# lucasnewman/f5-tts-mlx

Hardware: AMD Instinct MI355X
Metric: mel_frames_per_sec (higher is better)
Workload: dtype f16 (IEEE-half MFMA operands, fp32 accumulate / residual stream / LayerNorm / softmax state; meets the 1e-3 gate); 1 GPU; BASELINE configs[1]: F5-TTS 335M, 32-point euler (=62 DiT forwards, CFG), batch 1/GPU x 10 s (N=937) utterances, hipGraph=True; f16 (IEEE half) MFMA operands IN PLACE OF BASELINE's bf16 -- same width and MFMA rate, three more significand bits; plain bf16 fails the 1e-3 parity gate, see sub.b1_bf16; global_batch=1, seq_len=937, parallelism=dp1 (utterance sharding)

## Files before the change

f5_tts_mlx_amd/csrc/attention.hip:

```cpp
#include "attention.hpp"

namespace F5_NS {

__device__ __forceinline__ bool attn_block_map(const F5AttnArgs& p, int qrows, int& bh, int& qblk) {
    if (gridDim.y != 1) {
        bh = blockIdx.y;
        qblk = blockIdx.x;
        return true;
    }
    const int nqb = (p.seq_len + qrows - 1) / qrows;
    const int s = blockIdx.x >> 3;
    qblk = s % nqb;
    bh = (s / nqb) * 8 + (blockIdx.x & 7);
    return bh < p.B * p.H;
}

template <bool SCALE>
__device__ __forceinline__ void attn_pin_args(const F5AttnArgs& p) {
    if (SCALE)
        asm volatile("" ::"s"(p.qk[0]), "s"(p.vt[0]), "s"(p.out[0]), "s"(p.kv_len), "s"(p.B), "s"(p.H), "s"(p.seq_len), "s"(p.npad), "s"(p.ldqk),
                     "s"(p.ldo), "s"(p.dmodel), "s"(p.scale), "s"(p.out8));
    else
        asm volatile("" ::"s"(p.qk[0]), "s"(p.vt[0]), "s"(p.out[0]), "s"(p.kv_len), "s"(p.B), "s"(p.H), "s"(p.seq_len), "s"(p.npad), "s"(p.ldqk),
                     "s"(p.ldo), "s"(p.dmodel), "s"(p.out8));
// ... 775 lines not shown
    }

#define A2P_STEP(PH)                                                                                                    \
    if (j < T) {                                                                                                        \
        A2P_WAIT_TOP(j)                                                                                                 \
        attn_barrier();                                                                                                 \
        A2P_ISSUE_GROUP(j)                                                                                              \
        const int nv_ = kvlen - j * 64;                                                                                 \
         \
        attn2p_half<((PH) + 1) & 3, 0, (PH), 0>(ak, av, qf, fr_a, fr_b, s_a, s_b, o, mneg, p_b, p_a, l_run, hi, nv_);       \
        attn2p_half<((PH) + 1) & 3, 1, (PH), 1>(ak, av, qf, fr_b, fr_a, s_b, s_a, o, mneg, p_a, p_b, l_run, hi, nv_ - 32);  \
        ++j;                                                                                                            \
    }
    {
        int j = 0;
        for (int g = (T + 3) >> 2; g > 0; --g) {
            A2P_STEP(0)
            A2P_STEP(1)
            A2P_STEP(2)
            A2P_STEP(3)
        }
    }
#undef A2P_STEP
    {
        const uint32_t stv = (uint32_t)((T - 1) & 3) * (ATTN2P_TILE * 2);
        uint32_t avf[4];
#pragma unroll
        for (int i = 0; i < 4; ++i) avf[i] = av[i] + stv;
        a2p_load_frag<4, 0, 0, 0, 1>(fr_a[0], ak, avf);
        a2p_load_frag<5, 0, 0, 0, 1>(fr_a[1], ak, avf);
        a2p_load_frag<6, 0, 0, 0, 1>(fr_a[2], ak, avf);
        a2p_load_frag<7, 0, 0, 0, 1>(fr_a[3], ak, avf);
        asm volatile("s_waitcnt lgkmcnt(0)" : "+a"(fr_a[0]), "+a"(fr_a[1]), "+a"(fr_a[2]), "+a"(fr_a[3]));
#pragma unroll
        for (int g = 0; g < 4; ++g) {
            const int sp = g >> 1, db = g & 1;
#pragma unroll
            for (int qb = 0; qb < 2; ++qb) {
                const op16x8 pb = __builtin_bit_cast(op16x8, u32x4{p_b[qb][4 * sp], p_b[qb][4 * sp + 1], p_b[qb][4 * sp + 2], p_b[qb][4 * sp + 3]});
                a2p_mfma_o(o[qb][db], fr_a[g], pb);
            }
        }
    }
#undef A2P_WAIT_TOP
#undef A2P_ISSUE_GROUP
#undef A2P_ISSUE_V
#undef A2P_ISSUE_K
    asm volatile(A2P_PAD : "+a"(o[0][0]), "+a"(o[0][1]), "+a"(o[1][0]), "+a"(o[1][1]));

#pragma unroll
    for (int qb = 0; qb < 2; ++qb) attn_store_block<false>(p, o[qb], l_run[qb], rowbase, q0 + qb * 32 + lq, h, hi);
}

template <bool HP, int KS, int NST, bool FAST = false>
__global__ __launch_bounds__(256 * KS, 1) void f5_attn2s_kernel(F5AttnArgs p) {
    constexpr int NP = HP ? 2 : 1;
    constexpr int TILE = 64 * 64;
    constexpr int RING = NST * NP * 2 * TILE;
    static_assert(KS * RING * 2 <= 160 * 1024, "LDS budget");
    static_assert((KS - 1) * 4 * 34 * 64 * 4 <= KS * RING * 2, "merge area must fit in the rings");
    __shared__ __attribute__((aligned(16))) op16_t smem_all[KS * RING];

    attn_pin_args<true>(p);
    const int tid = threadIdx.x, lane = tid & 63;
    const int wave_all = __builtin_amdgcn_readfirstlane(tid >> 6);
    const int grp = wave_all >> 2, wave = wave_all & 3;
    const int tg = tid & 255;
    op16_t* smem = smem_all + grp * RING;
    const int hi = lane >> 5, lq = lane & 31;
    int bh, qblk;
    if (!attn_block_map(p, 128, bh, qblk)) return;
    const int b = bh / p.H, h = bh - b * p.H;
    const int q0 = qblk * 128 + wave * 32;
    const int kvlen = p.kv_len ? p.kv_len[b] : p.seq_len;
    const int ntile = (kvlen + 63) >> 6;
    const int nit = (ntile + KS - 1) / KS;
    const int ntg = ntile > grp ? (ntile - grp + KS - 1) / KS : 0;
    const size_t rowbase = (size_t)b * p.seq_len;

    op16x8 qf[NP][4];
    {
        int qr = q0 + lq;
        if (qr > p.seq_len - 1) qr = p.seq_len - 1;
#pragma unroll
        for (int pp = 0; pp < NP; ++pp)
#pragma unroll
            for (int ks = 0; ks < 4; ++ks)
                qf[pp][ks] = *reinterpret_cast<const op16x8*>(p.qk[pp] + (rowbase + qr) * p.ldqk + h * 64 + ks * 16 + hi * 8);
    }

    const op16_t* kptr[NP][2];
    const op16_t* vptr[NP][2];
    int krow[2], kcol[2], ldsoff[2];
#pragma unroll
    for (int i = 0; i < 2; ++i) {
        const int q_ = i * 256 + tg;
        const int srow = q_ >> 3;
        const int schunk = (q_ & 7) ^ ((srow >> 1) & 7);
        krow[i] = attn_kperm(srow);
        kcol[i] = p.dmodel + h * 64 + schunk * 8;
        ldsoff[i] = (i * 256 + wave * 64) * 8;
#pragma unroll
        for (int pp = 0; pp < NP; ++pp) {
            kptr[pp][i] = p.qk[pp] + (rowbase + grp * 64 + krow[i]) * p.ldqk + kcol[i];
            vptr[pp][i] = p.vt[pp] + ((size_t)bh * 64 + srow) * p.npad + grp * 64 + schunk * 8;
        }
    }
    const size_t kstep = (size_t)64 * KS * p.ldqk;
#define A2S_ISSUE(jj_)                                                                                       \
    {                                                                                                        \
        op16_t* st_ = smem + ((jj_) % NST) * (NP * 2 * TILE);                                                \
        const int gt_ = (jj_) * KS + grp;                                                                    \
        const bool tail_ = (gt_ * 64 + 63) > p.seq_len - 1;                                                  \
        _Pragma("unroll") for (int i = 0; i < 2; ++i) {                                                      \
            _Pragma("unroll") for (int pp = 0; pp < NP; ++pp) {                                              \
                const op16_t* ks_ = kptr[pp][i];                                                             \
                if (tail_) {                                                                                 \
                    int key_ = gt_ * 64 + krow[i];                                                           \
                    if (key_ > p.seq_len - 1) key_ = p.seq_len - 1;                                          \
                    ks_ = p.qk[pp] + (rowbase + key_) * p.ldqk + kcol[i];                                    \
                }                                                                                            \
                attn_glds16(ks_, st_ + (pp * 2) * TILE + ldsoff[i]);                                         \
                attn_glds16(vptr[pp][i], st_ + (pp * 2 + 1) * TILE + ldsoff[i]);                             \
                kptr[pp][i] += kstep;                                                                        \
                vptr[pp][i] += 64 * KS;                                                                      \
            }                                                                                                \
        }                                                                                                    \
    }

    f32x16 o[2];
#pragma unroll
    for (int e = 0; e < 16; ++e) {
        o[0][e] = 0.0f;
        o[1][e] = 0.0f;
    }
    float m_run = -INFINITY, l_run = 0.0f;
    const float c2 = p.q_prescaled ? 1.0f : p.scale * 1.4426950408889634f;

    if (ntg > 0) A2S_ISSUE(0);
    if (NST == 3 && ntg > 1) A2S_ISSUE(1);
    ATTN_PIN_Q(qf, NP, 4);

    for (int jj = 0; jj < nit; ++jj) {
        attn_wait_barrier(NST == 3 && jj + 1 < ntg);
        if (jj + NST - 1 < ntg) A2S_ISSUE(jj + NST - 1);
        if (jj >= ntg) continue;

        const op16_t* st = smem + (jj % NST) * (NP * 2 * TILE);
        const op16_t* sK = st;
        const op16_t* sV = st + TILE;
        const op16_t* sKl = st + (NP - 1) * 2 * TILE;
        const op16_t* sVl = st + (NP - 1) * 2 * TILE + TILE;

        f32x16 s[2];
        const int key0 = (jj * KS + grp) * 64;
#define A2S_QK()                                                                                             \
        {                                                                                                    \
            __builtin_amdgcn_s_setprio(1);                                                                   \
            _Pragma("unroll") for (int kb = 0; kb < 2; ++kb) {                                               \
                _Pragma("unroll") for (int e = 0; e < 16; ++e) s[kb][e] = 0.0f;                              \
                _Pragma("unroll") for (int ks = 0; ks < 4; ++ks) {                                           \
                    const int off = attn_swz(kb * 32 + lq, ks * 2 + hi);                                     \
                    const op16x8 a = *reinterpret_cast<const op16x8*>(&sK[off]);                             \
                    s[kb] = F5_MFMA32(a, qf[0][ks], s[kb], 0, 0, 0);                                         \
                    if (HP) {                                                                                \
                        const op16x8 al = *reinterpret_cast<const op16x8*>(&sKl[off]);                       \
                        s[kb] = F5_MFMA32(al, qf[0][ks], s[kb], 0, 0, 0);                                    \
                        s[kb] = F5_MFMA32(a, qf[NP - 1][ks], s[kb], 0, 0, 0);                                \
                    }                                                                                        \
                }                                                                                            \
            }                                                                                                \
            __builtin_amdgcn_s_setprio(0);                                                                   \
            if (key0 + 64 > kvlen) {                                                                         \
                _Pragma("unroll") for (int kb = 0; kb < 2; ++kb)                                             \
                    _Pragma("unroll") for (int r = 0; r < 16; ++r) {                                         \
                        const int key = key0 + kb * 32 + 16 * hi + r;                                        \
                        if (key >= kvlen) s[kb][r] = -INFINITY;                                              \
                    }                                                                                        \
            }                                                                                                \
        }
        A2S_QK();
        float psum = 0.0f;
        bool slow = !FAST || HP || jj == 0;
        if (!slow) {
            const float mc = m_run * c2;
            attn_f32x2 ps2 = {0.0f, 0.0f};
            ps2 = attn_exp_block(s[0], c2, mc, ps2);
            ps2 = attn_exp_block(s[1], c2, mc, ps2);
            psum = ps2[0] + ps2[1];
            slow = __any(!(psum <= ATTN_SUM_LIMIT));
            if (slow) A2S_QK();
        }
        if (slow) {
            float tmax = -INFINITY;
#pragma unroll
            for (int kb = 0; kb < 2; ++kb)
#pragma unroll
                for (int r = 0; r < 16; ++r) tmax = fmaxf(tmax, s[kb][r]);
            tmax = fmaxf(tmax, __shfl_xor(tmax, 32, 64));
            if (__any(tmax > m_run)) {
                const float m_new = fmaxf(m_run, tmax);
                const float alpha = __builtin_amdgcn_exp2f((m_run - m_new) * c2);
                m_run = m_new;
                l_run *= alpha;
#pragma unroll
                for (int e = 0; e < 16; ++e) {
                    o[0][e] *= alpha;
                    o[1][e] *= alpha;
                }
            }
            const float mc = m_run * c2;
            attn_f32x2 ps2 = {0.0f, 0.0f};
            ps2 = attn_exp_block(s[0], c2, mc, ps2);
            ps2 = attn_exp_block(s[1], c2, mc, ps2);
            psum = ps2[0] + ps2[1];
        }
        l_run += psum;
#undef A2S_QK

#pragma unroll
        for (int ks4 = 0; ks4 < 4; ++ks4) {
            const int kb = ks4 >> 1, sp = ks4 & 1;
            uint32_t pw[4], pwl[4];
#pragma unroll
            for (int e = 0; e < 4; ++e) {
                const float p0 = s[kb][8 * sp + 2 * e], p1 = s[kb][8 * sp + 2 * e + 1];
                pw[e] = f5_pack2_bounded(p0, p1);
                if (HP) pwl[e] = f5_pack2_lo(p0, p1);
            }
            const op16x8 pb = __builtin_bit_cast(op16x8, u32x4{pw[0], pw[1], pw[2], pw[3]});
            op16x8 pbl = pb;
            if (HP) pbl = __builtin_bit_cast(op16x8, u32x4{pwl[0], pwl[1], pwl[2], pwl[3]});
            __builtin_amdgcn_s_setprio(1);
#pragma unroll
            for (int db = 0; db < 2; ++db) {
                const int voff = attn_swz(db * 32 + lq, 4 * kb + 2 * hi + sp);
                const op16x8 a = *reinterpret_cast<const op16x8*>(&sV[voff]);
                o[db] = F5_MFMA32(a, pb, o[db], 0, 0, 0);
                if (HP) {
                    const op16x8 al = *reinterpret_cast<const op16x8*>(&sVl[voff]);
                    o[db] = F5_MFMA32(al, pb, o[db], 0, 0, 0);
                    o[db] = F5_MFMA32(a, pbl, o[db], 0, 0, 0);
                }
            }
            __builtin_amdgcn_s_setprio(0);
        }
    }
#undef A2S_ISSUE

    __syncthreads();
    float* mrg = reinterpret_cast<float*>(smem_all);
    if (HP || !p.out8) {
        constexpr int Q = 32 / KS, NPK = 2 + 32 - Q;
        constexpr int SLD = 64 + 8;
        static_assert(KS * 4 * NPK * 64 * 4 + (HP ? 0 : 128 * SLD * 2) <= KS * RING * 2, "merge area + output staging fit in the rings");
        float* mine = mrg + (size_t)((grp * 4 + wave) * NPK) * 64 + lane;
        mine[0] = m_run;
        mine[64] = l_run;
#pragma unroll
        for (int g = 0; g < KS; ++g)
            if (grp == g) {
#pragma unroll
                for (int i = 0; i < 32; ++i)
                    if (i / Q != g) mine[(2 + (i < g * Q ? i : i - Q)) * 64] = o[i >> 4][i & 15];
            }
        __syncthreads();
        const float* src[KS];
        float mg[KS];
#pragma unroll
        for (int g = 0; g < KS; ++g) {
            src[g] = mrg + (size_t)((g * 4 + wave) * NPK) * 64 + lane;
            mg[g] = src[g][0];
        }
        float m_all = mg[0];
#pragma unroll
        for (int g = 1; g < KS; ++g) m_all = fmaxf(m_all, mg[g]);
        float ag[KS];
#pragma unroll
        for (int g = 0; g < KS; ++g) ag[g] = __builtin_amdgcn_exp2f((mg[g] - m_all) * c2);
        float l_all = __builtin_fmaf(src[0][64], ag[0], src[1][64] * ag[1]);
#pragma unroll
        for (int g = 2; g < KS; ++g) l_all = __builtin_fmaf(src[g][64], ag[g], l_all);
        float own[Q];
#pragma unroll
        for (int g = 0; g < KS; ++g)
            if (grp == g) {
#pragma unroll
                for (int j = 0; j < Q; ++j) {
                    const int i = g * Q + j;
                    float w[KS];
#pragma unroll
                    for (int k = 0; k < KS; ++k) {
                        w[k] = ag[k];
                        asm volatile("" : "+v"(w[k]));
                    }
                    float x[KS];
#pragma unroll
                    for (int k = 0; k < KS; ++k) x[k] = k == g ? o[i >> 4][i & 15] : src[k][(2 + (i < k * Q ? i : i - Q)) * 64];
                    float acc;
                    if (KS == 2) {
// ... 44 lines not shown
#pragma unroll
        for (int db = 0; db < 2; ++db)
#pragma unroll
            for (int e = 0; e < 16; ++e) dst[(2 + db * 16 + e) * 64] = o[db][e];
    }
    __syncthreads();
    if (grp > 0) return;
    float m_all = m_run;
#pragma unroll
    for (int g = 1; g < KS; ++g) m_all = fmaxf(m_all, mrg[(size_t)((g - 1) * 4 + wave) * 34 * 64 + lane]);
    {
        const float a0 = __builtin_amdgcn_exp2f((m_run - m_all) * c2);
        l_run *= a0;
#pragma unroll
        for (int e = 0; e < 16; ++e) {
            o[0][e] *= a0;
            o[1][e] *= a0;
        }
    }
#pragma unroll
    for (int g = 1; g < KS; ++g) {
        const float* src = mrg + (size_t)((g - 1) * 4 + wave) * 34 * 64 + lane;
        const float ag = __builtin_amdgcn_exp2f((src[0] - m_all) * c2);
        l_run += src[64] * ag;
#pragma unroll
        for (int db = 0; db < 2; ++db)
#pragma unroll
            for (int e = 0; e < 16; ++e) o[db][e] += src[(2 + db * 16 + e) * 64] * ag;
    }

    const float l_tot = l_run + __shfl_xor(l_run, 32, 64);
    const float inv = 1.0f / l_tot;
    const int qr = q0 + lq;
    if (!HP && p.out8) {
        if (qr < p.seq_len) attn_store_f8(p, o, inv, rowbase + qr, h, hi);
    } else if (qr < p.seq_len) {
#pragma unroll
        for (int db = 0; db < 2; ++db)
#pragma unroll
            for (int rg = 0; rg < 4; ++rg) {
                const int d = db * 32 + 8 * rg + 4 * hi;
                const float v0 = o[db][rg * 4 + 0] * inv, v1 = o[db][rg * 4 + 1] * inv;
                const float v2 = o[db][rg * 4 + 2] * inv, v3 = o[db][rg * 4 + 3] * inv;
                const size_t off = (rowbase + qr) * p.ldo + h * 64 + d;
                *reinterpret_cast<u32x2*>(p.out[0] + off) = u32x2{f5_pack2_bounded(v0, v1), f5_pack2_bounded(v2, v3)};
                if (HP && p.out[1])
                    *reinterpret_cast<u32x2*>(p.out[1] + off) = u32x2{f5_pack2_lo(v0, v1), f5_pack2_lo(v2, v3)};
            }
    }
}

int f5_attn_wide = -1;
int f5_attn_kvsplit = -1;
int f5_attn_pipe = 0;

static dim3 attn_grid(const F5AttnArgs& a, int qrows) {
    const int nqb = f5_cdiv(a.seq_len, qrows);
    return dim3(nqb * 8 * f5_cdiv(a.B * a.H, 8), 1);
}

static F5AttnKernel attn_route(const F5AttnArgs& a) {
    int ks = f5_attn_kvsplit;
    if (ks < 0) {
        const long wgs = (long)f5_cdiv(a.seq_len, 128) * a.B * a.H;
        const int ntile = f5_cdiv(a.seq_len, 64);
        ks = (wgs <= 160 && ntile >= 8) ? 4 : ((wgs <= 320 && ntile >= 4) ? 2 : 1);
    }
    if (!a.hp && ks <= 1 &&
        (f5_attn_wide >= 1 || (f5_attn_wide < 0 && (long)f5_cdiv(a.seq_len, 256) * a.B * a.H >= 512))) {
        const bool pipe = (a.pipe < 0 ? f5_attn_pipe : a.pipe) && a.q_prescaled;
        return pipe ? F5A_V2P : (a.q_prescaled ? F5A_V2F_PRE : F5A_V2F);
    }
    if (ks > 1) return a.hp ? F5A_V2S_HP : (ks >= 4 ? F5A_V2S_KS4 : F5A_V2S_KS2);
    return a.hp ? F5A_V2_HP : F5A_V2;
}

static int attn_launch(const F5AttnArgs& a, hipStream_t stream, int& reached) {
    F5_REQUIRE(a.B > 0 && a.H > 0 && a.seq_len > 0, "attention: bad shape");
    F5_REQUIRE(a.npad % 64 == 0 && a.npad >= a.seq_len, "attention: npad must be a multiple of 64 and >= seq_len");
    F5_REQUIRE(a.ldqk % 8 == 0 && a.ldo % 4 == 0, "attention: bad leading dims");
    F5_REQUIRE(a.qk[0] && a.vt[0] && (a.out[0] || a.out8), "attention: null pointer");
    F5_REQUIRE(!a.out8 || (!a.hp && a.out8s && a.ldo8 % 4 == 0),
               "attention: fp8 output needs the bf16 ring kernels");
    F5_REQUIRE(!a.hp || (a.qk[1] && a.vt[1] && a.out[1]), "attention: bf16x3 needs lo buffers");
    const F5AttnKernel k = attn_route(a);
    const dim3 grid = attn_grid(a, 128), gw = attn_grid(a, 256);
    switch (k) {
        case F5A_V2_HP: hipLaunchKernelGGL(f5_attn2_kernel<true>, grid, dim3(256), 0, stream, a); break;
        case F5A_V2: hipLaunchKernelGGL(f5_attn2_kernel<false>, grid, dim3(256), 0, stream, a); break;
        case F5A_V2F_PRE: hipLaunchKernelGGL(f5_attn2f_kernel<true>, gw, dim3(256), 0, stream, a); break;
        case F5A_V2F: hipLaunchKernelGGL(f5_attn2f_kernel<false>, gw, dim3(256), 0, stream, a); break;
        case F5A_V2P: hipLaunchKernelGGL(f5_attn2p_kernel, gw, dim3(256), 0, stream, a); break;
        case F5A_V2S_HP: hipLaunchKernelGGL((f5_attn2s_kernel<true, 2, 2>), grid, dim3(512), 0, stream, a); break;
        case F5A_V2S_KS2: hipLaunchKernelGGL((f5_attn2s_kernel<false, 2, 3, true>), grid, dim3(512), 0, stream, a); break;
        case F5A_V2S_KS4: hipLaunchKernelGGL((f5_attn2s_kernel<false, 4, 2, true>), grid, dim3(1024), 0, stream, a); break;
        default: break;
    }
    F5_LAUNCH_CHECK();
    reached = k;
    return 0;
}

int f5_launch_attention(const F5AttnArgs& a, hipStream_t stream) {
    int reached = F5A_NONE;
    const int rc = attn_launch(a, stream, reached);
    f5dbg::last_attn_kernel = rc == 0 ? (reached | (a.out8 ? F5A_OUT8 : 0)) : F5A_NONE;
    return rc;
}
}
```

f5_tts_mlx_amd/csrc/common.hpp:

```cpp
#pragma once
#include <hip/hip_runtime.h>
#include <stdint.h>
#include <stdio.h>
#include <string.h>

typedef float f32x16 __attribute__((ext_vector_type(16)));
typedef float f32x4 __attribute__((ext_vector_type(4)));
typedef unsigned short u16;
typedef uint32_t u32x4 __attribute__((ext_vector_type(4)));
typedef uint32_t u32x2 __attribute__((ext_vector_type(2)));

#define F5_WAVE 64

#include "gemm_route.hpp"

void f5_set_error(const char* fmt, ...);
#define F5_HIP_CHECK(expr)                                                                        \
    do {                                                                                          \
        hipError_t _e = (expr);                                                                   \
        if (_e != hipSuccess) {                                                                   \
            f5_set_error("%s failed: %s (%s:%d)", #expr, hipGetErrorString(_e), __FILE__, __LINE__); \
            return 1;                                                                             \
        }                                                                                         \
    } while (0)
#define F5_LAUNCH_CHECK() F5_HIP_CHECK(hipGetLastError())
#define F5_REQUIRE(cond, ...)                                                                     \
    do {                                                                                          \
        if (!(cond)) {                                                                            \
            f5_set_error(__VA_ARGS__);                                                            \
            return 2;                                                                             \
        }                                                                                         \
    } while (0)

namespace f5dbg {
extern int last_gemm_kernel;
}
enum F5AttnKernel {
    F5A_NONE = 0,
    F5A_V2_HP,
    F5A_V2,
    F5A_V2F_PRE,
    F5A_V2F,
    F5A_V2P,
    F5A_V2S_HP,
    F5A_V2S_KS2,
    F5A_V2S_KS4,
    F5A_OUT8 = 16
};
namespace f5dbg {
extern int last_attn_kernel;
}
enum F5ConvPosKernel {
    F5CP_NONE = 0,
    F5CP_1,
    F5CP_2,
    F5CP_4,
    F5CP_HP1,
    F5CP_HP2,
    F5CP_RING,
    F5CP_XCD = 16
};
namespace f5dbg {
extern int last_convpos_kernel;
}

inline u16 f5_f2bf_bits(float f) {
    uint32_t u;
    memcpy(&u, &f, 4);
    if ((u & 0x7fffffffu) > 0x7f800000u) return (u16)((u >> 16) | 0x40);
    uint32_t r = u + 0x7fffu + ((u >> 16) & 1u);
    return (u16)(r >> 16);
}
inline float f5_bf_bits2f(u16 h) {
    uint32_t u = ((uint32_t)h) << 16;
    float f;
    memcpy(&f, &u, 4);
    return f;
}
inline u16 f5_f2h_bits(float f) {
    uint32_t u;
    memcpy(&u, &f, 4);
    const u16 sign = (u16)((u >> 16) & 0x8000u);
    const uint32_t a = u & 0x7fffffffu;
    if (a > 0x7f800000u) return (u16)(sign | 0x7e00u);
    if (a >= 0x477ff000u) return (u16)(sign | 0x7bffu);
    if (a < 0x33000001u) return sign;
    const int e = (int)(a >> 23) - 127;
    uint32_t m = (a & 0x7fffffu) | 0x800000u;
    int shift = e >= -14 ? 13 : 13 + (-14 - e);
    const uint32_t half = 1u << (shift - 1), mask = (1u << shift) - 1u;
    uint32_t q = m >> shift;
    const uint32_t rem = m & mask;
    if (rem > half || (rem == half && (q & 1u))) ++q;
    const uint32_t he = e >= -14 ? (uint32_t)(e + 15 - 1) << 10 : 0u;
    return (u16)(sign | (u16)(he + q));
}
inline float f5_h_bits2f(u16 h) {
    const uint32_t sign = ((uint32_t)h & 0x8000u) << 16;
    const uint32_t e = (h >> 10) & 31u, m = h & 0x3ffu;
// ... 99 lines not shown
```

f5_tts_mlx_amd/csrc/engine.hip:

```cpp
#include <stdarg.h>

#include <cmath>

#include <string>
#include <vector>

#include "../../include/f5tts_hip.h"
#include "host_common.hpp"

static Ops g_ops;

static thread_local char g_err[1024] = "";
void f5_set_error(const char* fmt, ...) {
    va_list ap;
    va_start(ap, fmt);
    vsnprintf(g_err, sizeof(g_err), fmt, ap);
    va_end(ap);
}
extern "C" const char* f5_last_error(void) { return g_err; }
extern "C" int f5_version(void) { return 1; }

struct MatF8 {
    size_t q = 0, s = 0;
    int rows = 0, ld = 0;
// ... 1288 lines not shown
    memcpy(words.data(), t_rows_host, (size_t)c.B * 4);
    RC(f5_launch_stage_words(words.data(), words.size(), c.p<uint32_t>(c.w.rscal), s));
    const Ops& K = c.ops;
    RC(run_prep(c, 1));
    RC(K.pack_x(c.p<float>(c.w.traj), c.pb(c.w.xin, 0), c.pb(c.w.xin, 1), (int)M1, mel, s));
    RC(run_dit(c, 0));
    RC(f5_launch_copy_words(c.ws + c.w.vel, pred, M1 * mel, s));
    if (null_pred && c.nb == 2) RC(f5_launch_copy_words(c.ws + c.w.vel + M1 * mel * 4, null_pred, M1 * mel, s));
    return 0;
}

extern "C" int f5_dit_forward_dual(f5_engine* e, const f5_sample_args* a, const float* x, const float* t_rows_host, float* pred,
                                   float* null_pred, float* text_pred, void* stream) {
    RC(check_args(e, a));
    F5_REQUIRE(x && pred, "null pointer");
    F5_REQUIRE(t_rows_host != nullptr, "f5_dit_forward_dual: t_rows is null");
    RC(check_dual_route(e, "f5_dit_forward_dual"));
    for (int b = 0; b < a->B; ++b) F5_REQUIRE(std::isfinite(t_rows_host[b]), "f5_dit_forward_dual: t_rows[%d] is not finite", b);
    hipStream_t s = (hipStream_t)stream;
    f5_sample_args a2 = *a;
    a2.steps = 2;
    a2.method = F5_EULER;
    Ctx c = make_ctx(e, &a2, s);
    const float on = 1.0f;
    ctx_to_dual(c, &a2, &on, &on, 1);
    F5_REQUIRE(a->workspace_bytes >= c.w.total_rows, "f5_dit_forward_dual: workspace too small: %zu < %zu (f5_workspace_bytes_dual)",
               a->workspace_bytes, c.w.total_rows);
    if (ln_fold_state(c) < 0) return 2;
    const int mel = e->cfg.mel_dim;
    const size_t M1 = (size_t)c.B * c.N;
    SatScope sat(e->prec == F5_PREC_F16 && e->opt.sat_check, c.p<int>(c.w.status));
    std::vector<float> tnfe(1, t_rows_host[0]), dts(1, 0.0f);
    RC(stage_inputs(c, &a2, x, tnfe, dts));
    std::vector<uint32_t> words(c.w.rscal_words, 0u);
    memcpy(words.data(), t_rows_host, (size_t)c.B * 4);
    RC(f5_launch_stage_words(words.data(), words.size(), c.p<uint32_t>(c.w.rscal), s));
    const Ops& K = c.ops;
    RC(run_prep(c, 1));
    RC(K.pack_x(c.p<float>(c.w.traj), c.pb(c.w.xin, 0), c.pb(c.w.xin, 1), (int)M1, mel, s));
    RC(run_dit(c, 0));
    float* outs[3] = {pred, null_pred, text_pred};
    for (int br = 0; br < 3; ++br)
        if (outs[br]) RC(f5_launch_copy_words(c.ws + c.w.vel + (size_t)br * M1 * mel * 4, outs[br], M1 * mel, s));
    return 0;
}

#define F5_DECL_KNOB(v) namespace f5bf { extern int v; } namespace f5hf { extern int v; }
#define F5_SET_BOTH(v, x) do { f5bf::v = (x); f5hf::v = (x); ++g_knob_epoch; } while (0)
#define F5_SET_ROUTE_KNOB(v, x) do { f5dbg::gemm_knobs.v = (x); ++g_knob_epoch; } while (0)
F5_DECL_KNOB(f5_convpos_tps)
F5_DECL_KNOB(f5_convpos_xcd_map)
F5_DECL_KNOB(f5_attn_wide)
F5_DECL_KNOB(f5_attn_kvsplit)
F5_DECL_KNOB(f5_attn_pipe)
F5_DECL_KNOB(f5_gemm_order)
F5_DECL_KNOB(f5_gemm_nband)
F5_DECL_KNOB(f5_gemm_debug_flags)
extern "C" int f5_op_set_operand_type(int fp16) {
    F5_REQUIRE(fp16 == 0 || fp16 == 1, "operand type must be 0 (bf16) or 1 (fp16)");
    g_ops.h = fp16 != 0;
    return 0;
}
extern "C" int f5_op_get_operand_type(void) { return g_ops.h ? 1 : 0; }
extern "C" uint16_t f5_debug_f2h_bits(float f) { return f5_f2h_bits(f); }
extern "C" float f5_debug_h_bits2f(uint16_t h) { return f5_h_bits2f(h); }
extern "C" uint16_t f5_debug_f2bf_bits(float f) { return f5_f2bf_bits(f); }
extern "C" int f5_debug_set_convpos_tps(int v) {
    F5_REQUIRE(v == 0 || v == 1 || v == 2 || v == 4 || v == 8, "conv-pos taps per pipeline step must be 0 (auto), 1, 2, 4 or 8 (the ring kernel)");
    F5_SET_BOTH(f5_convpos_tps, v);
    return 0;
}
extern "C" int f5_debug_set_convpos_xcd_map(int on) {
    F5_SET_BOTH(f5_convpos_xcd_map, on ? 1 : 0);
    return 0;
}
static void warn_defaults_only(const char* hook, const char* option) {
    if (g_live_engines > 0)
        fprintf(stderr, "[f5tts_hip] %s changes the default of NEW engines only: %d engine(s) already exist and keep their value "
                        "(use f5_engine_set_option(e, \"%s\", v) for those)\n", hook, g_live_engines, option);
}
extern "C" int f5_debug_set_ln_fusion(int on) {
    warn_defaults_only("f5_debug_set_ln_fusion", "ln_fusion");
    g_default_options.fuse_ln = on ? 1 : 0;
    return 0;
}
extern "C" int f5_debug_set_qkv_transposed(int on) {
    warn_defaults_only("f5_debug_set_qkv_transposed", "qkv_transposed");
    g_default_options.qkv_tr = on ? 1 : 0;
    return 0;
}
extern "C" int f5_debug_set_q_premul(int on) {
    warn_defaults_only("f5_debug_set_q_premul", "q_premul");
    g_default_options.q_premul = on ? 1 : 0;
    return 0;
}
extern "C" int f5_debug_set_attn_wide(int v) {
    F5_REQUIRE(v >= -1 && v <= 1, "attention wide-workgroup switch must be -1 (auto), 0 or 1 (256-query workgroups)");
    F5_SET_BOTH(f5_attn_wide, v);
    return 0;
}
extern "C" int f5_debug_set_attn_pipe(int v) {
    F5_REQUIRE(v == 0 || v == 1, "attention pipelining switch must be 0 (v2f) or 1 (v2p: in-wave software pipeline, one wave per SIMD)");
    F5_SET_BOTH(f5_attn_pipe, v);
    return 0;
}
extern "C" int f5_debug_set_attn_kvsplit(int v) {
    F5_REQUIRE(v == -1 || v == 1 || v == 2 || v == 4, "attention KV split must be -1 (auto), 1, 2 or 4");
    F5_SET_BOTH(f5_attn_kvsplit, v);
    return 0;
}
extern "C" int f5_debug_set_gemm_qkv_tile(int v) {
    F5_REQUIRE(v == 0 || v == 1 || v == 12 || v == 13 || v == 14, "small-M QKV tile must be 0 (auto), 1 (small tiles), 12 / 13 (8-wave 128x256 ring) or 14 (role-split 128x256)");
    F5_SET_ROUTE_KNOB(qkv_tile, v);
    return 0;
}
extern "C" int f5_debug_set_gemm_nband(int v) {
    F5_REQUIRE(v >= 0 && v <= 16, "column-tile band width of the 256x256 tile numbering must be 0 (n fastest) .. 16");
    F5_SET_BOTH(f5_gemm_nband, v);
    return 0;
}
extern "C" int f5_debug_set_gemm_ring(int v) {
    F5_SET_ROUTE_KNOB(ring, v ? 1 : 0);
    return 0;
}
extern "C" int f5_debug_set_gemm_order(int v) {
    F5_REQUIRE(v >= 0 && v <= 3, "gemm order must be 0 (auto), 1 (n fastest), 2 (m fastest) or 3 (band-major where it applies)");
    F5_SET_BOTH(f5_gemm_order, v);
    return 0;
}
extern "C" int f5_debug_set_gemm_flags(int v) {
    F5_SET_BOTH(f5_gemm_debug_flags, v);
    return 0;
}
namespace f5dbg {
int last_gemm_kernel = 0;
int last_attn_kernel = 0;
int last_convpos_kernel = 0;
}
static int copy_name(const std::string& s, char* buf, int n) {
    if (buf != nullptr && n > 0) {
        strncpy(buf, s.c_str(), (size_t)n - 1);
        buf[n - 1] = 0;
    }
    return (int)s.size();
}
extern "C" int f5_debug_last_gemm_kernel(char* buf, int n) {
    return copy_name(f5_gemm_kernel_name(f5dbg::last_gemm_kernel), buf, n);
}
extern "C" int f5_debug_last_attn_kernel(char* buf, int n) {
    static const char* const names[] = {"", "f5_attn2_kernel<true,0>", "f5_attn2_kernel<false,0>", "f5_attn2f_kernel<true>", "f5_attn2f_kernel<false>",
                                        "f5_attn2p_kernel", "f5_attn2s_kernel<true,2,2>", "f5_attn2s_kernel<false,2,3,true>",
                                        "f5_attn2s_kernel<false,4,2,true>"};
    const int k = f5dbg::last_attn_kernel & (F5A_OUT8 - 1);
    std::string s = k <= F5A_V2S_KS4 ? names[k] : "";
    if (k != F5A_NONE && (f5dbg::last_attn_kernel & F5A_OUT8)) s += "+f8";
    return copy_name(s, buf, n);
}
static std::string convpos_kernel_name(int word) {
    static const char* const names[] = {"", "f5_convpos_kernel<false,1>", "f5_convpos_kernel<false,2>", "f5_convpos_kernel<false,4>",
                                        "f5_convpos_kernel<true,1>", "f5_convpos_kernel<true,2>", "f5_convpos_ring_kernel"};
    const int k = word & (F5CP_XCD - 1);
    std::string s = k <= F5CP_RING ? names[k] : "";
    if (k != F5CP_NONE && (word & F5CP_XCD)) s += "+xcd";
    return s;
}
extern "C" int f5_debug_last_convpos_kernel(char* buf, int n) { return copy_name(convpos_kernel_name(f5dbg::last_convpos_kernel), buf, n); }
extern "C" int f5_debug_convpos_route(int B, int seq_len, int groups, int nseg, char* buf, int n) {
    F5_REQUIRE(B > 0 && seq_len > 0 && groups > 0 && (nseg == 1 || nseg == 3), "convpos route: bad shape");
    copy_name(convpos_kernel_name(f5bf::f5_convpos_route(B, seq_len, groups, nseg)), buf, n);
    return 0;
}
extern "C" int f5_debug_gemm_route(int epi, int M, int N, int nseg, int seq_len, int variant_bits, int debug_flags, char* name, int n, int* facts) {
    F5_REQUIRE(epi >= EPI_F32 && epi <= EPI_GELU_ERF_BF16 && M >= 1 && N >= 1, "gemm route: bad epilogue %d or shape M=%d N=%d", epi, M, N);
    const F5GemmQuery q = {epi, M, N, nseg, seq_len, (variant_bits & 1) != 0, (variant_bits & 2) != 0, (unsigned)(variant_bits >> 2) & 7u,
                           debug_flags | f5bf::f5_gemm_debug_flags};
    const F5GemmRoute r = f5_gemm_route(q);
    if (facts != nullptr) *facts = (r.staged ? 1 : 0) | (r.fold_small ? 2 : 0) | (r.ln_fusable ? 4 : 0);
    if (r.kernel == F5K_NONE) {
        f5_set_error("%s", r.refused);
        return -1;
    }
    return copy_name(f5_gemm_kernel_name(f5_gemm_reached(r.kernel, q)), name, n);
}
extern "C" int f5_debug_set_gemm_tile(int sel) {
    F5_REQUIRE(sel >= 0 && sel <= 14, "gemm tile override must be 0 (auto) .. 14");
    F5_REQUIRE(sel != 7, "gemm tile 7 does not exist (tiles are 0 .. 6 and 8 .. 14)");
    F5_SET_ROUTE_KNOB(tile, sel);
    return 0;
}

static struct {
    const float* next_scale = nullptr;
    op16_t* x16 = nullptr;
    float* stats_out = nullptr;
    const float* row_shift = nullptr;
    float* ln_mean_out = nullptr;
    const float* rowf = nullptr;
    const float* c1 = nullptr;
    const float* c2 = nullptr;
} g_op_fold;
extern "C" int f5_debug_set_op_fold_producer(const float* next_scale, void* x16_out, float* stats_out, const float* row_shift) {
    g_op_fold.next_scale = next_scale;
    g_op_fold.x16 = (op16_t*)x16_out;
    g_op_fold.stats_out = stats_out;
    g_op_fold.row_shift = row_shift;
    return 0;
}
// ... 525 lines not shown
```

f5_tts_mlx_amd/engine.py:

```python
from __future__ import annotations

import ctypes as C
import os
import warnings
from concurrent.futures import ThreadPoolExecutor
from pathlib import Path
from typing import Dict, Optional, Sequence

import numpy as np
import torch

from .weights import DiTConfig, check_weights

_LIB_PATH = Path(os.environ["F5TTS_HIP_LIB"]).resolve() if os.environ.get("F5TTS_HIP_LIB") else Path(__file__).resolve().parent / "csrc" / "libf5tts_hip.so"
_lib = None

METHODS = {"euler": 0, "midpoint": 1, "rk4": 2}
PRECISIONS = {"bf16": 0, "bf16x3": 1, "mxfp8": 2, "f16": 3}
GRAPH_MODES = {False: 0, True: 1, "off": 0, "on": 1, "auto": 2}


def operand_dtype(precision: str) -> torch.dtype:
    return torch.float16 if precision == "f16" else torch.bfloat16

# ... 56 lines not shown
        return int(t.shape[0]), None
    if t.ndim == 2 and t.shape[0] != B:
        raise ValueError(f"per-row time grid: expected {B} rows, got {t.shape[0]}")
    cfg = np.asarray(cfg_strength, dtype=np.float32)
    if cfg_seq and cfg.shape != (B,):
        raise ValueError(f"per-row cfg_strength: expected {B} values, got shape {cfg.shape}")
    steps = int(t.shape[-1])
    t_rows = np.ascontiguousarray(np.broadcast_to(t, (B, steps)), dtype=np.float32)
    cfg_rows = np.ascontiguousarray(np.broadcast_to(cfg, (B,)), dtype=np.float32)
    return steps, (t_rows, cfg_rows)


def _rows_slice(t, cfg_strength, b0: int, b1: int):
    t = np.asarray(t, dtype=np.float32)
    return (t[b0:b1] if t.ndim == 2 else t), (cfg_strength if np.ndim(cfg_strength) == 0 else list(cfg_strength)[b0:b1])


def _audio_slice(audio_cfg_strength, b0: int, b1: int):
    if audio_cfg_strength is None or np.ndim(audio_cfg_strength) == 0:
        return audio_cfg_strength
    return list(np.asarray(audio_cfg_strength, dtype=np.float32)[b0:b1])


def _plan_of(rows):
    return False if rows is None else ("dual" if len(rows) == 3 else True)


def library_path() -> Path:
    return _LIB_PATH


def load_library() -> C.CDLL:
    global _lib
    if _lib is not None:
        return _lib
    if not _LIB_PATH.exists():
        raise RuntimeError(
            f"HIP extension not built: {_LIB_PATH} is missing. Run `python -c 'import __graft_entry__ as g; g.build()'` "
            "(or f5_tts_mlx_amd/csrc/build.sh). There is no CPU fallback.")
    lib = C.CDLL(str(_LIB_PATH))
    lib.f5_last_error.restype = C.c_char_p
    lib.f5_version.restype = C.c_int
    lib.f5_op_grn_scratch_floats.restype = C.c_size_t
    lib.f5_engine_destroy.restype = None
    lib.f5_debug_f2h_bits.restype = C.c_uint16
    lib.f5_debug_f2h_bits.argtypes = [C.c_float]
    lib.f5_debug_f2bf_bits.restype = C.c_uint16
    lib.f5_debug_f2bf_bits.argtypes = [C.c_float]
    lib.f5_debug_h_bits2f.restype = C.c_float
    lib.f5_debug_h_bits2f.argtypes = [C.c_uint16]
    lib.f5_debug_last_convpos_kernel.argtypes = [C.c_char_p, C.c_int]
    if hasattr(lib, "f5_debug_convpos_route"):
        lib.f5_debug_convpos_route.argtypes = [C.c_int] * 4 + [C.c_char_p, C.c_int]
    lib.f5_op_noise_from_bits.argtypes = [C.c_void_p, C.c_size_t, C.c_void_p, C.c_void_p]
    lib.f5_sample_edit.argtypes = [C.c_void_p, C.c_void_p, C.c_void_p, C.c_void_p]
    for name, types in (("f5_sample_rows", [C.c_void_p] * 4), ("f5_dit_forward_rows", [C.c_void_p] * 7),
                        ("f5_workspace_bytes_rows", [C.c_void_p] + [C.c_int] * 5 + [C.c_void_p]),
                        ("f5_sample_dual", [C.c_void_p] * 4), ("f5_dit_forward_dual", [C.c_void_p] * 8),
                        ("f5_workspace_bytes_dual", [C.c_void_p] + [C.c_int] * 5 + [C.c_void_p]),
                        ("f5_op_ode_stage_dual", [C.c_void_p] * 7 + [C.c_int, C.c_int, C.c_float, C.c_float, C.c_int] + [C.c_void_p] * 7
                         + [C.c_int, C.c_int, C.c_void_p]),
                        ("f5_op_pack_cond_text_dual", [C.c_void_p] * 5 + [C.c_int] * 4 + [C.c_void_p]),
                        ("f5_op_pack_cond_text_dual_keep", [C.c_void_p] * 5 + [C.c_int] * 4 + [C.c_void_p]),
                        ("f5_op_resid_gate_ln_rows", [C.c_void_p] * 8 + [C.c_int] * 4 + [C.c_size_t, C.c_void_p]),
                        ("f5_op_ode_stage_rows", [C.c_void_p] * 5 + [C.c_int, C.c_int, C.c_float, C.c_float, C.c_int] + [C.c_void_p] * 7
                         + [C.c_int, C.c_int, C.c_void_p]),
                        ("f5_op_ln_modulate_f8", [C.c_void_p] * 5 + [C.c_int, C.c_int, C.c_float, C.c_void_p]),
                        ("f5_op_quantize_mx_bf16", [C.c_void_p, C.c_int, C.c_void_p, C.c_int, C.c_void_p, C.c_int, C.c_int, C.c_void_p]),
                        ("f5_op_qkv_rope_f8", [C.c_void_p] * 9 + [C.c_int] * 7 + [C.c_float, C.c_void_p])):
        if hasattr(lib, name):
            getattr(lib, name).argtypes = types
    lib.f5_op_wave_patch.argtypes = [C.c_void_p, C.c_void_p, C.c_void_p, C.c_void_p, C.c_void_p, C.c_int, C.c_int64, C.c_int64, C.c_int,
                                     C.c_int, C.c_void_p]
    lib.f5_wave_block_energy.argtypes = [C.c_void_p, C.c_int, C.c_int64, C.c_void_p, C.c_int, C.c_void_p, C.c_int, C.c_void_p]
    lib.f5_mel_spectrogram_ragged.argtypes = [C.c_void_p, C.c_int, C.c_int64, C.c_void_p, C.c_void_p, C.c_void_p, C.c_void_p, C.c_void_p,
                                              C.c_int, C.c_int, C.c_int, C.c_void_p, C.c_int, C.c_void_p]
    _lib = lib
    return lib


def check(rc: int, what: str = "") -> None:
    if rc != 0:
        msg = load_library().f5_last_error().decode("utf-8", "replace")
        if msg.startswith("Unknown method"):
            raise ValueError(msg)
        raise RuntimeError(f"{what or 'f5 call'} failed (rc={rc}): {msg}")


def ptr(t: Optional[torch.Tensor]) -> C.c_void_p:
    return C.c_void_p(0 if t is None else t.data_ptr())


def stream_ptr(device: torch.device) -> C.c_void_p:
    return C.c_void_p(torch.cuda.current_stream(device).cuda_stream)


def noise_normal(seeds: Sequence[int], durations: Sequence[int], N: int, mel: int, device: torch.device) -> torch.Tensor:
    lib = load_library()
    B = len(durations)
    if len(seeds) != B:
        raise ValueError("one seed per batch element")
    device = torch.device(device)
    y0 = torch.empty((B, int(N), int(mel)), dtype=torch.float32, device=device)
    CH = 256
    scratch = torch.empty(3 * min(B, CH), dtype=torch.int32, device=device)
    with torch.cuda.device(device):
# ... 495 lines not shown
```

include/f5tts_hip.h:

```cpp
#ifndef F5TTS_HIP_H
#define F5TTS_HIP_H

#include <stddef.h>
#include <stdint.h>

#ifdef __cplusplus
extern "C" {
#endif

typedef struct f5_engine f5_engine;

typedef struct f5_config {
    int32_t dim;
    int32_t depth;
    int32_t heads;
    int32_t dim_head;
    int32_t ff_dim;
    int32_t mel_dim;
    int32_t text_num_embeds;
    int32_t text_dim;
    int32_t text_ff_dim;
    int32_t conv_layers;
    int32_t conv_pos_kernel;
    int32_t conv_pos_groups;
// ... 141 lines not shown
int f5_op_pack_x(const float* y, void* out_hi, void* out_lo, int rows, int mel_dim, void* stream);
int f5_op_splice(const float* cond, const float* y, const int32_t* lens, float* out, int B, int seq_len, int mel_dim, void* stream);
int f5_op_pack_cond_text_keep(const float* cond, const uint8_t* keep, const float* text_emb, void* out_hi, void* out_lo, int B,
                              int seq_len, int mel_dim, int dt, int null_keeps_cond, void* stream);
int f5_op_splice_keep(const float* cond, const float* y, const uint8_t* keep, float* out, int B, int seq_len, int mel_dim, void* stream);
int f5_op_pack_cond_text_dual(const float* cond, const int32_t* lens, const float* text_emb, void* out_hi, void* out_lo, int B, int seq_len,
                              int mel_dim, int dt, void* stream);
int f5_op_pack_cond_text_dual_keep(const float* cond, const uint8_t* keep, const float* text_emb, void* out_hi, void* out_lo, int B,
                                   int seq_len, int mel_dim, int dt, void* stream);
int f5_op_gather_frames(const float* src, const int32_t* src_idx, float* cond_out, uint8_t* keep_out, int B, int n_src, int seq_len,
                        int mel_dim, void* stream);
int f5_op_rowkeep(const int32_t* dur, uint8_t* keep, int nbatch, int seq_len, void* stream);
int f5_op_copy_words(const void* src, void* dst, size_t nwords, void* stream);
int f5_op_stage_words(const uint32_t* host_words, size_t nwords, uint32_t* dst, void* stream);
int f5_op_zero_vt_pad(void* vt, size_t rows, int seq_len, int npad, void* stream);

int f5_noise_normal(const uint64_t* seeds, int B, const int32_t* durations, int N, int mel, float* y0, void* scratch_words,
                    void* stream);
int f5_op_noise_from_bits(const uint32_t* bits_dev, size_t n, float* out, void* stream);

int f5_op_gemm_resid_gate(const void* a_hi, const void* a_lo, const void* w_hi, const void* w_lo, const float* bias,
                          const float* gate, const uint8_t* rowkeep, float* x, int M, int N, int K, int lda, int ldw, int ldx,
                          int nseg, void* stream);
int f5_op_gemm_resid_gate_ln(const void* a_hi, const void* a_lo, const void* w_hi, const void* w_lo, const float* bias,
                             const float* gate, const uint8_t* rowkeep, float* x, const float* ln_scale, const float* ln_shift,
                             void* h_hi, void* h_lo, int* counters, int M, int N, int K, int lda, int ldw, int nseg, void* stream);
int f5_op_gemm_addrows(const void* a_hi, const void* a_lo, const void* w_hi, const void* w_lo, const float* addrows,
                       int a_row_mod, float* out_f32, void* out_hi, void* out_lo, int M, int N, int K, int lda, int ldw, int ldo,
                       int nseg, void* stream);
int f5_op_layernorm(const float* x, const float* w, const float* b, float* out_f32, void* out_hi, void* out_lo, int rows,
                    int dim, void* stream);
int f5_op_im2col7(const float* x, void* out_hi, void* out_lo, int nbatch, int seq_len, int channels, void* stream);
int f5_op_istft(const float* x, int ldx, const float* window, float* frames_scratch, float* wave, int nframes, int n_fft,
                int hop, void* stream);

uint16_t f5_debug_f2h_bits(float f);
float f5_debug_h_bits2f(uint16_t h);
uint16_t f5_debug_f2bf_bits(float f);
int f5_debug_set_gemm_tile(int sel);
int f5_debug_last_gemm_kernel(char* buf, int n);
int f5_debug_last_attn_kernel(char* buf, int n);
int f5_debug_last_convpos_kernel(char* buf, int n);
int f5_debug_convpos_route(int B, int seq_len, int groups, int nseg, char* buf, int n);
int f5_debug_gemm_route(int epi, int M, int N, int nseg, int seq_len, int variant_bits, int debug_flags, char* name, int n, int* facts);
int f5_debug_set_gemm_flags(int v);
int f5_debug_set_gemm_order(int v);
int f5_debug_set_gemm_ring(int v);
int f5_debug_set_gemm_qkv_tile(int sel);
int f5_debug_set_gemm_nband(int n);
int f5_debug_set_convpos_tps(int taps);
int f5_debug_set_convpos_xcd_map(int on);
int f5_debug_set_attn_wide(int v);
int f5_debug_set_attn_kvsplit(int v);
int f5_debug_set_attn_pipe(int v);
int f5_debug_set_ln_fusion(int on);
int f5_debug_set_qkv_transposed(int on);
int f5_debug_set_q_premul(int on);
int f5_debug_set_op_fold_producer(const float* next_scale, void* x16_out, float* stats_out, const float* row_shift);
int f5_op_fold_rows(const float* stats, int nslice, int M, float* rowf, float* row_shift, void* stream);
int f5_debug_set_op_ln_mean_out(float* mean_out);
int f5_debug_set_op_fold_consumer(const float* rowf, const float* c1, const float* c2);
int f5_debug_set_op_fold_stats(const float* stats, int ld, const float* shift, float* mean_out);
int f5_debug_set_op_sat_flag(int* flag);
int f5_debug_set_op_fold_overflow_flag(int* flag);
int f5_op_fold_consts(const void* w_hi, int ldw, const float* bias, const float* scale, const float* shift, size_t vec_stride, int nvec,
                      float* c1, float* c2, size_t out_stride, int N, int K, void* stream);
int f5_debug_set_op_rope_tables_g4(const float* tq, const float* tk);
int f5_debug_set_op_q_premul(float factor);

int f5_op_quantize_mx(const float* x, int ldx, void* q, int ldq, void* scales, int rows, int cols, void* stream);
int f5_op_quantize_mx_bf16(const void* x16, int ldx, void* q, int ldq, void* scales, int rows, int cols, void* stream);
int f5_op_ln_modulate_f8(const float* x, const float* scale, const float* shift, void* q, void* q_scales, int rows, int dim, float eps,
                         void* stream);
int f5_op_gemm_f8(const void* a8, const void* a_scales, const void* w8, const void* w_scales, const float* bias,
                  const float* gate, const uint8_t* rowkeep, float* out_f32, void* out_bf, void* out8, void* out8_scales,
                  int M, int N, int K, int lda8, int ldw8, int ldo, int epi, void* stream);
int f5_op_qkv_rope_f8(const void* a8, const void* a_scales, const void* w8, const void* w_scales, const float* bias, const float* rope_cos,
                      const float* rope_sin, void* qk, void* vt, int B, int seq_len, int npad, int heads, int dmodel, int lda8, int ldw8,
                      float q_premul, void* stream);

int f5_mel_spectrogram_batch(const float* wave, int B, int64_t L, const float* window, const float* filterbank, int n_fft, int hop,
                             int n_mels, float* out, void* stream);
int f5_mel_spectrogram(const float* wave, int64_t L, const float* window, const float* filterbank, int n_fft, int hop,
                       int n_mels, float* out, void* stream);
int f5_mel_spectrogram_ragged(const float* wave, int B, int64_t L, const int32_t* begin_dev, const int32_t* lens_dev,
                              const float* gain_dev , const float* window, const float* filterbank, int n_fft, int hop,
                              int n_mels, float* out, int N, void* stream);
int f5_wave_block_energy(const float* wave, int B, int64_t L, const int32_t* lens_dev, int block, float* energy, int nblk,
                         void* stream);
int f5_resample_batch(const float* wave, int B, int64_t L, const float* taps, const int32_t* first, int o, int n, int T, int width,
                      float* out, int64_t L_out, void* stream);

int f5_op_wave_patch(const float* gen, const float* src, const int32_t* segs_host, const float* fade, float* out, int B, int64_t L,
                     int64_t Ls, int S, int F, void* stream);

typedef struct f5_vocoder f5_vocoder;
typedef struct f5_vocos_config {
    int32_t n_mels;
    int32_t dim;
    int32_t intermediate_dim;
    int32_t num_layers;
    int32_t n_fft;
    int32_t hop_length;
} f5_vocos_config;
int f5_vocoder_create(const f5_vocos_config* cfg, int precision, f5_vocoder** out);
void f5_vocoder_destroy(f5_vocoder* v);
// ... 67 lines not shown
```

Before: 13940 mel-frames/s.

## Add skewed two-group attention schedule and V-fragment preloading behind knob

Adds a skewed variant of the two-group KV-split attention kernel in which group 1 runs its PV MFMAs one iteration behind its QK step. The two groups then issue different work at once, so softmax and MFMA phases overlap across groups. The route is gated by a new f5_attn_skew knob that defaults to auto, and the auto value is compiled off. It also adds VPRE, enabled by default, which loads V fragments from LDS into registers right after QK so the reads overlap the softmax exp work, at the cost of more VGPRs. Ablation macros (A2S_ABL) are added for probing and are off by default.

```diff
diff --git a/f5_tts_mlx_amd/csrc/attention.hip b/f5_tts_mlx_amd/csrc/attention.hip
--- a/f5_tts_mlx_amd/csrc/attention.hip
+++ b/f5_tts_mlx_amd/csrc/attention.hip
@@ -851,8 +851,27 @@
     for (int qb = 0; qb < 2; ++qb) attn_store_block<false>(p, o[qb], l_run[qb], rowbase, q0 + qb * 32 + lq, h, hi);
 }
 
-template <bool HP, int KS, int NST, bool FAST = false>
+#ifndef A2S_ABL
+#define A2S_ABL 0
+#endif
+#ifndef A2S_SKEW_NST
+#define A2S_SKEW_NST 4
+#endif
+#ifndef A2S_VPRE
+#define A2S_VPRE 1
+#endif
+__device__ __forceinline__ f32x16 a2s_mfma(const op16x8& a, const op16x8& b, f32x16 c) {
+    if (A2S_ABL & 4) {
+        asm volatile("" : "+v"(c) : "v"(a), "v"(b));
+        return c;
+    }
+    return F5_MFMA32(a, b, c, 0, 0, 0);
+}
+#define A2S_FRAG(ptr_) ((A2S_ABL & 8) ? qf[0][0] : *reinterpret_cast<const op16x8*>(ptr_))
+
+template <bool HP, int KS, int NST, bool FAST = false, bool SKEW = false>
 __global__ __launch_bounds__(256 * KS, 1) void f5_attn2s_kernel(F5AttnArgs p) {
+    static_assert(!SKEW || (KS == 2 && !HP && FAST && (NST == 3 || NST == 4)), "the skewed schedule is the two-group one-pass FAST kernel's");
     constexpr int NP = HP ? 2 : 1;
     constexpr int TILE = 64 * 64;
     constexpr int RING = NST * NP * 2 * TILE;
@@ -936,13 +955,42 @@
     float m_run = -INFINITY, l_run = 0.0f;
     const float c2 = p.q_prescaled ? 1.0f : p.scale * 1.4426950408889634f;
 
+    constexpr bool VPRE = A2S_VPRE && !HP && KS == 2;
+    op16x8 vf[8];
+    const int pd = !SKEW ? NST - 1 : ((NST == 3 && grp == 1) ? 1 : 2);
+    uint32_t pk[16];
+#define A2S_PV(sV_)                                                                                          \
+    _Pragma("unroll") for (int ks4 = 0; ks4 < 4; ++ks4) {                                                    \
+        const int kb = ks4 >> 1, sp = ks4 & 1;                                                               \
+        const op16x8 pb = __builtin_bit_cast(op16x8, u32x4{pk[4 * ks4], pk[4 * ks4 + 1], pk[4 * ks4 + 2], pk[4 * ks4 + 3]}); \
+        __builtin_amdgcn_s_setprio(1);                                                                       \
+        _Pragma("unroll") for (int db = 0; db < 2; ++db) {                                                   \
+            const int voff = attn_swz(db * 32 + lq, 4 * kb + 2 * hi + sp);                                   \
+            const op16x8 a = VPRE ? vf[ks4 * 2 + db] : A2S_FRAG(&(sV_)[voff]);                               \
+            o[db] = a2s_mfma(a, pb, o[db]);                                                                  \
+        }                                                                                                    \
+        __builtin_amdgcn_s_setprio(0);                                                                       \
+    }
+
     if (ntg > 0) A2S_ISSUE(0);
-    if (NST == 3 && ntg > 1) A2S_ISSUE(1);
+    if (pd == 2 && ntg > 1) A2S_ISSUE(1);
     ATTN_PIN_Q(qf, NP, 4);
 
-    for (int jj = 0; jj < nit; ++jj) {
-        attn_wait_barrier(NST == 3 && jj + 1 < ntg);
-        if (jj + NST - 1 < ntg) A2S_ISSUE(jj + NST - 1);
+    for (int jj = 0; jj < ((A2S_ABL & 1) ? 0 : nit); ++jj) {
+        if (A2S_ABL & 16) {
+            if (pd == 2 && jj + 1 < ntg) {
+                asm volatile("s_waitcnt vmcnt(4)" ::: "memory");
+            } else {
+                asm volatile("s_waitcnt vmcnt(0)" ::: "memory");
+            }
+        } else {
+            attn_wait_barrier(pd == 2 && jj + 1 < ntg);
+        }
+        if (jj + pd < ntg) A2S_ISSUE(jj + pd);
+        if (SKEW && grp == 1 && jj >= 1 && jj <= ntg) {
+            const op16_t* sVp = smem + ((jj - 1) % NST) * (NP * 2 * TILE) + TILE;
+            A2S_PV(sVp);
+        }
         if (jj >= ntg) continue;
 
         const op16_t* st = smem + (jj % NST) * (NP * 2 * TILE);
@@ -960,12 +1008,12 @@
                 _Pragma("unroll") for (int e = 0; e < 16; ++e) s[kb][e] = 0.0f;                              \
                 _Pragma("unroll") for (int ks = 0; ks < 4; ++ks) {                                           \
                     const int off = attn_swz(kb * 32 + lq, ks * 2 + hi);                                     \
-                    const op16x8 a = *reinterpret_cast<const op16x8*>(&sK[off]);                             \
-                    s[kb] = F5_MFMA32(a, qf[0][ks], s[kb], 0, 0, 0);                                         \
+                    const op16x8 a = A2S_FRAG(&sK[off]);                                                     \
+                    s[kb] = a2s_mfma(a, qf[0][ks], s[kb]);                                                   \
                     if (HP) {                                                                                \
-                        const op16x8 al = *reinterpret_cast<const op16x8*>(&sKl[off]);                       \
-                        s[kb] = F5_MFMA32(al, qf[0][ks], s[kb], 0, 0, 0);                                    \
-                        s[kb] = F5_MFMA32(a, qf[NP - 1][ks], s[kb], 0, 0, 0);                                \
+                        const op16x8 al = A2S_FRAG(&sKl[off]);                                               \
+                        s[kb] = a2s_mfma(al, qf[0][ks], s[kb]);                                              \
+                        s[kb] = a2s_mfma(a, qf[NP - 1][ks], s[kb]);                                          \
                     }                                                                                        \
                 }                                                                                            \
             }                                                                                                \
@@ -979,9 +1027,16 @@
             }                                                                                                \
         }
         A2S_QK();
+        if (VPRE) {
+#pragma unroll
+            for (int ks4 = 0; ks4 < 4; ++ks4)
+#pragma unroll
+                for (int db = 0; db < 2; ++db) vf[ks4 * 2 + db] = A2S_FRAG(&sV[attn_swz(db * 32 + lq, 4 * (ks4 >> 1) + 2 * hi + (ks4 & 1))]);
+            __builtin_amdgcn_sched_barrier(0);
+        }
         float psum = 0.0f;
-        bool slow = !FAST || HP || jj == 0;
-        if (!slow) {
+        bool slow = !(A2S_ABL & 2) && (!FAST || HP || jj == 0);
+        if (!(A2S_ABL & 2) && !slow) {
             const float mc = m_run * c2;
             attn_f32x2 ps2 = {0.0f, 0.0f};
             ps2 = attn_exp_block(s[0], c2, mc, ps2);
@@ -1016,7 +1071,22 @@
         }
         l_run += psum;
 #undef A2S_QK
-
+        if (VPRE) {
+#pragma unroll
+            for (int i = 0; i < 8; ++i) asm volatile("" ::"v"(vf[i]));
+        }
+
+        if (SKEW) {
+#pragma unroll
+            for (int ks4 = 0; ks4 < 4; ++ks4)
+#pragma unroll
+                for (int e = 0; e < 4; ++e) {
+                    const float p0 = s[ks4 >> 1][8 * (ks4 & 1) + 2 * e], p1 = s[ks4 >> 1][8 * (ks4 & 1) + 2 * e + 1];
+                    pk[4 * ks4 + e] = (A2S_ABL & 2) ? __float_as_uint(p0) : f5_pack2_bounded(p0, p1);
+                }
+            if (grp == 0) A2S_PV(sV);
+            continue;
+        }
 #pragma unroll
         for (int ks4 = 0; ks4 < 4; ++ks4) {
             const int kb = ks4 >> 1, sp = ks4 & 1;
@@ -1024,7 +1094,7 @@
 #pragma unroll
             for (int e = 0; e < 4; ++e) {
                 const float p0 = s[kb][8 * sp + 2 * e], p1 = s[kb][8 * sp + 2 * e + 1];
-                pw[e] = f5_pack2_bounded(p0, p1);
+                pw[e] = (A2S_ABL & 2) ? __float_as_uint(p0) : f5_pack2_bounded(p0, p1);
                 if (HP) pwl[e] = f5_pack2_lo(p0, p1);
             }
             const op16x8 pb = __builtin_bit_cast(op16x8, u32x4{pw[0], pw[1], pw[2], pw[3]});
@@ -1034,17 +1104,23 @@
 #pragma unroll
             for (int db = 0; db < 2; ++db) {
                 const int voff = attn_swz(db * 32 + lq, 4 * kb + 2 * hi + sp);
-                const op16x8 a = *reinterpret_cast<const op16x8*>(&sV[voff]);
-                o[db] = F5_MFMA32(a, pb, o[db], 0, 0, 0);
+                const op16x8 a = VPRE ? vf[ks4 * 2 + db] : A2S_FRAG(&sV[voff]);
+                o[db] = a2s_mfma(a, pb, o[db]);
                 if (HP) {
-                    const op16x8 al = *reinterpret_cast<const op16x8*>(&sVl[voff]);
-                    o[db] = F5_MFMA32(al, pb, o[db], 0, 0, 0);
-                    o[db] = F5_MFMA32(a, pbl, o[db], 0, 0, 0);
+                    const op16x8 al = A2S_FRAG(&sVl[voff]);
+                    o[db] = a2s_mfma(al, pb, o[db]);
+                    o[db] = a2s_mfma(a, pbl, o[db]);
                 }
             }
             __builtin_amdgcn_s_setprio(0);
         }
     }
+    if (SKEW && grp == 1 && ntg > 0 && ntg == nit && !(A2S_ABL & 1)) {
+        const op16_t* sVp = smem + ((ntg - 1) % NST) * (NP * 2 * TILE) + TILE;
+        A2S_PV(sVp);
+    }
+    if (A2S_ABL & 1) asm volatile("s_waitcnt vmcnt(0)" ::: "memory");
+#undef A2S_PV
 #undef A2S_ISSUE
 
     __syncthreads();
@@ -1195,6 +1271,7 @@
 
 int f5_attn_wide = -1;
 int f5_attn_kvsplit = -1;
+int f5_attn_skew = -1;
 int f5_attn_pipe = 0;
 
 static dim3 attn_grid(const F5AttnArgs& a, int qrows) {
@@ -1202,6 +1279,10 @@
     return dim3(nqb * 8 * f5_cdiv(a.B * a.H, 8), 1);
 }
 
+#ifndef A2S_SKEW_AUTO
+#define A2S_SKEW_AUTO 0
+#endif
+constexpr bool ATTN_SKEW_AUTO = A2S_SKEW_AUTO != 0;
 static F5AttnKernel attn_route(const F5AttnArgs& a) {
     int ks = f5_attn_kvsplit;
     if (ks < 0) {
@@ -1214,7 +1295,11 @@
         const bool pipe = (a.pipe < 0 ? f5_attn_pipe : a.pipe) && a.q_prescaled;
         return pipe ? F5A_V2P : (a.q_prescaled ? F5A_V2F_PRE : F5A_V2F);
     }
-    if (ks > 1) return a.hp ? F5A_V2S_HP : (ks >= 4 ? F5A_V2S_KS4 : F5A_V2S_KS2);
+    if (ks > 1) {
+        if (a.hp) return F5A_V2S_HP;
+        if (ks >= 4) return F5A_V2S_KS4;
+        return (f5_attn_skew > 0 || (f5_attn_skew < 0 && ATTN_SKEW_AUTO)) ? F5A_V2S_KS2_SKEW : F5A_V2S_KS2;
+    }
     return a.hp ? F5A_V2_HP : F5A_V2;
 }
 
@@ -1237,6 +1322,7 @@
         case F5A_V2S_HP: hipLaunchKernelGGL((f5_attn2s_kernel<true, 2, 2>), grid, dim3(512), 0, stream, a); break;
         case F5A_V2S_KS2: hipLaunchKernelGGL((f5_attn2s_kernel<false, 2, 3, true>), grid, dim3(512), 0, stream, a); break;
         case F5A_V2S_KS4: hipLaunchKernelGGL((f5_attn2s_kernel<false, 4, 2, true>), grid, dim3(1024), 0, stream, a); break;
+        case F5A_V2S_KS2_SKEW: hipLaunchKernelGGL((f5_attn2s_kernel<false, 2, A2S_SKEW_NST, true, true>), grid, dim3(512), 0, stream, a); break;
         default: break;
     }
     F5_LAUNCH_CHECK();
diff --git a/f5_tts_mlx_amd/csrc/common.hpp b/f5_tts_mlx_amd/csrc/common.hpp
--- a/f5_tts_mlx_amd/csrc/common.hpp
+++ b/f5_tts_mlx_amd/csrc/common.hpp
@@ -45,6 +45,7 @@
     F5A_V2S_HP,
     F5A_V2S_KS2,
     F5A_V2S_KS4,
+    F5A_V2S_KS2_SKEW,
     F5A_OUT8 = 16
 };
 namespace f5dbg {
diff --git a/f5_tts_mlx_amd/csrc/engine.hip b/f5_tts_mlx_amd/csrc/engine.hip
--- a/f5_tts_mlx_amd/csrc/engine.hip
+++ b/f5_tts_mlx_amd/csrc/engine.hip
@@ -1364,6 +1364,7 @@
 F5_DECL_KNOB(f5_convpos_xcd_map)
 F5_DECL_KNOB(f5_attn_wide)
 F5_DECL_KNOB(f5_attn_kvsplit)
+F5_DECL_KNOB(f5_attn_skew)
 F5_DECL_KNOB(f5_attn_pipe)
 F5_DECL_KNOB(f5_gemm_order)
 F5_DECL_KNOB(f5_gemm_nband)
@@ -1421,6 +1422,11 @@
     F5_SET_BOTH(f5_attn_kvsplit, v);
     return 0;
 }
+extern "C" int f5_debug_set_attn_skew(int v) {
+    F5_REQUIRE(v >= -1 && v <= 1, "attention skew switch must be -1 (auto), 0 (lock-step two-group kernel) or 1 (skewed where the two-group one-pass kernel is the route)");
+    F5_SET_BOTH(f5_attn_skew, v);
+    return 0;
+}
 extern "C" int f5_debug_set_gemm_qkv_tile(int v) {
     F5_REQUIRE(v == 0 || v == 1 || v == 12 || v == 13 || v == 14, "small-M QKV tile must be 0 (auto), 1 (small tiles), 12 / 13 (8-wave 128x256 ring) or 14 (role-split 128x256)");
     F5_SET_ROUTE_KNOB(qkv_tile, v);
@@ -1462,9 +1468,9 @@
 extern "C" int f5_debug_last_attn_kernel(char* buf, int n) {
     static const char* const names[] = {"", "f5_attn2_kernel<true,0>", "f5_attn2_kernel<false,0>", "f5_attn2f_kernel<true>", "f5_attn2f_kernel<false>",
                                         "f5_attn2p_kernel", "f5_attn2s_kernel<true,2,2>", "f5_attn2s_kernel<false,2,3,true>",
-                                        "f5_attn2s_kernel<false,4,2,true>"};
+                                        "f5_attn2s_kernel<false,4,2,true>", "f5_attn2s_kernel<false,2,4,true,true>"};
     const int k = f5dbg::last_attn_kernel & (F5A_OUT8 - 1);
-    std::string s = k <= F5A_V2S_KS4 ? names[k] : "";
+    std::string s = k <= F5A_V2S_KS2_SKEW ? names[k] : "";
     if (k != F5A_NONE && (f5dbg::last_attn_kernel & F5A_OUT8)) s += "+f8";
     return copy_name(s, buf, n);
 }
diff --git a/f5_tts_mlx_amd/engine.py b/f5_tts_mlx_amd/engine.py
--- a/f5_tts_mlx_amd/engine.py
+++ b/f5_tts_mlx_amd/engine.py
@@ -132,6 +132,8 @@
     lib.f5_debug_last_convpos_kernel.argtypes = [C.c_char_p, C.c_int]
     if hasattr(lib, "f5_debug_convpos_route"):
         lib.f5_debug_convpos_route.argtypes = [C.c_int] * 4 + [C.c_char_p, C.c_int]
+    if hasattr(lib, "f5_debug_set_attn_skew"):
+        lib.f5_debug_set_attn_skew.argtypes = [C.c_int]
     lib.f5_op_noise_from_bits.argtypes = [C.c_void_p, C.c_size_t, C.c_void_p, C.c_void_p]
     lib.f5_sample_edit.argtypes = [C.c_void_p, C.c_void_p, C.c_void_p, C.c_void_p]
     for name, types in (("f5_sample_rows", [C.c_void_p] * 4), ("f5_dit_forward_rows", [C.c_void_p] * 7),
diff --git a/include/f5tts_hip.h b/include/f5tts_hip.h
--- a/include/f5tts_hip.h
+++ b/include/f5tts_hip.h
@@ -217,6 +217,7 @@
 int f5_debug_set_convpos_xcd_map(int on);
 int f5_debug_set_attn_wide(int v);
 int f5_debug_set_attn_kvsplit(int v);
+int f5_debug_set_attn_skew(int v);
 int f5_debug_set_attn_pipe(int v);
 int f5_debug_set_ln_fusion(int on);
 int f5_debug_set_qkv_transposed(int on);
```

Result: no change. 13900 mel-frames/s (-0.3%).
